# Renmusxd/PyIsingMonteCarlo

Measured on AMD Instinct MI355X. Metric: spin-flip attempts/s (whole node), 4096^2 2D Ising, higher is better.
Workload: dtype u32; 1 GPU; c2: 4096x4096 periodic Ising J=-1 beta=0.4407, 256 replicas/GPU, checkerboard Metropolis, bit-packed spins, Philox4x32-10; replicas_per_gpu=256, parallelism=replicas x1

## Files before the change

### pyisingmontecarlo_amd/csrc/lattice_kernels.hpp

```cpp
#pragma once
#include "philox.hpp"
#include <type_traits>

namespace isingmc {

struct LatGeom {
    uint32_t W, H;
    uint32_t wpr;
    uint32_t wpp;
    uint32_t nquads;
    int32_t cols_log2;
};

struct LatThr {
    uint64_t T3, T4;
};

#ifndef ISINGMC_N_PLANES
#define ISINGMC_N_PLANES 7
#endif
constexpr int N_PLANES = ISINGMC_N_PLANES;
constexpr int THR_BITS = N_PLANES + 32;

__device__ __forceinline__ uint32_t sel4(uint4 v, uint32_t i)
{
    return i == 0 ? v.x : i == 1 ? v.y : i == 2 ? v.z : v.w;
}

struct QuadNbr {
    uint32_t up[4], dn[4], ce[4], si[4];
};

template <bool UNI>
__device__ __forceinline__ void thread_to_quad(const LatGeom &g, uint32_t gid, uint32_t &Q, uint32_t &y,
                                               uint32_t &xw)
{
    if constexpr (UNI) {
        const uint32_t cl = uint32_t(g.cols_log2), col = gid & ((1u << cl) - 1);
        if (cl >= 6) {
            y = gid >> cl;
        } else {
            const uint32_t wave = gid >> 6, j = (gid & 63u) >> cl;
            y = ((wave >> 1) << (7 - cl)) + 2 * j + (wave & 1u);
        }
        Q = (y << cl) + col;
        xw = 4 * col;
    } else {
        Q = gid;
        y = (4 * Q) / g.wpr;
        xw = 4 * Q - y * g.wpr;
    }
}

struct PtrPlanes {
    uint32_t *own;
    const uint32_t *oth;
    __device__ __forceinline__ uint4 own4(uint32_t w) const { return *reinterpret_cast<const uint4 *>(own + w); }
    __device__ __forceinline__ uint4 oth4(uint32_t w) const { return *reinterpret_cast<const uint4 *>(oth + w); }
    __device__ __forceinline__ uint32_t own1(uint32_t w) const { return own[w]; }
    __device__ __forceinline__ uint32_t oth1(uint32_t w) const { return oth[w]; }
    __device__ __forceinline__ void store4(uint32_t w, uint4 v) const { *reinterpret_cast<uint4 *>(own + w) = v; }
    __device__ __forceinline__ void store1(uint32_t w, uint32_t v) const { own[w] = v; }
};

struct BufPlanes {
    __amdgpu_buffer_rsrc_t rsrc;
    uint32_t own_off, oth_off;
    typedef uint32_t u32x4 __attribute__((ext_vector_type(4)));
    __device__ __forceinline__ uint4 ld4(uint32_t byte_off) const
    {
        const u32x4 v = __builtin_amdgcn_raw_buffer_load_b128(rsrc, byte_off, 0, 0);
        return make_uint4(v.x, v.y, v.z, v.w);
    }
    __device__ __forceinline__ uint4 own4(uint32_t w) const { return ld4(own_off + 4 * w); }
    __device__ __forceinline__ uint4 oth4(uint32_t w) const { return ld4(oth_off + 4 * w); }
    __device__ __forceinline__ uint32_t own1(uint32_t w) const { return __builtin_amdgcn_raw_buffer_load_b32(rsrc, own_off + 4 * w, 0, 0); }
    __device__ __forceinline__ uint32_t oth1(uint32_t w) const { return __builtin_amdgcn_raw_buffer_load_b32(rsrc, oth_off + 4 * w, 0, 0); }
    __device__ __forceinline__ void store4(uint32_t w, uint4 v) const
    {
        __builtin_amdgcn_raw_buffer_store_b128(u32x4{v.x, v.y, v.z, v.w}, rsrc, own_off + 4 * w, 0, 0);
    }
    __device__ __forceinline__ void store1(uint32_t w, uint32_t v) const { __builtin_amdgcn_raw_buffer_store_b32(v, rsrc, own_off + 4 * w, 0, 0); }
};

__device__ __forceinline__ void side_words(QuadNbr &n, bool odd)
{
    const uint32_t sw = n.si[0];
    if (odd) {
        n.si[0] = (n.ce[0] >> 1) | (n.ce[1] << 31);
        n.si[1] = (n.ce[1] >> 1) | (n.ce[2] << 31);
        n.si[2] = (n.ce[2] >> 1) | (n.ce[3] << 31);
        n.si[3] = (n.ce[3] >> 1) | (sw << 31);
    } else {
        n.si[3] = (n.ce[3] << 1) | (n.ce[2] >> 31);
        n.si[2] = (n.ce[2] << 1) | (n.ce[1] >> 31);
        n.si[1] = (n.ce[1] << 1) | (n.ce[0] >> 31);
        n.si[0] = (n.ce[0] << 1) | (sw >> 31);
    }
}

template <bool VEC, bool UNI, typename Mem>
__device__ __forceinline__ void load_quad(const Mem &mem, const LatGeom &g,
                                          uint32_t colour, uint32_t Q, uint32_t y, uint32_t xw, uint32_t own[4],
                                          QuadNbr &n, uint32_t widx[4])
{
    if constexpr (VEC) {
        const uint32_t w0 = 4 * Q;
        const uint32_t yu = (y == 0 ? g.H : y) - 1, yd = (y + 1 == g.H) ? 0 : y + 1;
        bool odd = (y + colour) & 1u;
        if constexpr (UNI) odd = __builtin_amdgcn_readfirstlane(uint32_t(odd));
        const uint32_t sx = odd ? (xw + 4 == g.wpr ? 0 : xw + 4) : (xw == 0 ? g.wpr : xw) - 1;
        const auto row_base = [&](uint32_t row) { return UNI ? row << (uint32_t(g.cols_log2) + 2) : row * g.wpr; };
        const uint4 o4 = mem.own4(w0);
        const uint4 c4 = mem.oth4(w0);
        const uint4 u4 = mem.oth4(row_base(yu) + xw);
        const uint4 d4 = mem.oth4(row_base(yd) + xw);
        const uint32_t sw = mem.oth1(row_base(y) + sx);
        own[0] = o4.x; own[1] = o4.y; own[2] = o4.z; own[3] = o4.w;
        n.ce[0] = c4.x; n.ce[1] = c4.y; n.ce[2] = c4.z; n.ce[3] = c4.w;
        n.up[0] = u4.x; n.up[1] = u4.y; n.up[2] = u4.z; n.up[3] = u4.w;
        n.dn[0] = d4.x; n.dn[1] = d4.y; n.dn[2] = d4.z; n.dn[3] = d4.w;
        n.si[0] = sw;
        side_words(n, odd);
#pragma unroll
        for (int q = 0; q < 4; q++) widx[q] = w0 + q;
    } else {
#pragma unroll
        for (int q = 0; q < 4; q++) {
            const uint32_t w = 4 * Q + q;
            const uint32_t yy = w / g.wpr, xx = w - yy * g.wpr;
            const uint32_t yu = (yy == 0 ? g.H : yy) - 1, yd = (yy + 1 == g.H) ? 0 : yy + 1;
            const uint32_t row = yy * g.wpr;
            widx[q] = w;
            own[q] = mem.own1(w);
            n.ce[q] = mem.oth1(w);
            n.up[q] = mem.oth1(yu * g.wpr + xx);
            n.dn[q] = mem.oth1(yd * g.wpr + xx);
            if ((yy + colour) & 1) {
                const uint32_t nxt = mem.oth1(row + (xx + 1 == g.wpr ? 0 : xx + 1));
                n.si[q] = (n.ce[q] >> 1) | (nxt << 31);
            } else {
                const uint32_t prv = mem.oth1(row + (xx == 0 ? g.wpr : xx) - 1);
                n.si[q] = (n.ce[q] << 1) | (prv >> 31);
            }
        }
    }
}

template <bool PMJ>
__device__ __forceinline__ void bond_masks(const uint32_t own, const QuadNbr &n, int q,
                                           const uint32_t *__restrict__ jneg, uint32_t wpp,
                                           uint32_t widx, uint32_t jneg_uniform, uint32_t &a0,
                                           uint32_t &a1, uint32_t &a2, uint32_t &a3)
{
    if constexpr (PMJ) {
        a0 = own ^ n.up[q] ^ jneg[widx];
        a1 = own ^ n.dn[q] ^ jneg[wpp + widx];
        a2 = own ^ n.ce[q] ^ jneg[2 * wpp + widx];
        a3 = own ^ n.si[q] ^ jneg[3 * wpp + widx];
    } else {
        const uint32_t o = own ^ jneg_uniform;
        a0 = o ^ n.up[q];
        a1 = o ^ n.dn[q];
        a2 = o ^ n.ce[q];
        a3 = o ^ n.si[q];
    }
}

struct QuadState {
    uint32_t eq3[4], eq4[4], lt[4], und[4];
};

struct ThrBits {
    uint32_t hi3, hi4;
    uint32_t lo3, lo4;
    bool all3, all4;
    bool any_all;
};

__device__ __forceinline__ ThrBits thr_bits(const LatThr thr)
{
    ThrBits b;
    const uint32_t h3 = __builtin_amdgcn_readfirstlane(uint32_t(thr.T3 >> 32));
    const uint32_t h4 = __builtin_amdgcn_readfirstlane(uint32_t(thr.T4 >> 32));
    b.all3 = (h3 >> N_PLANES) != 0;
    b.all4 = (h4 >> N_PLANES) != 0;
    b.any_all = ((h3 | h4) >> N_PLANES) != 0;
    b.hi3 = h3 & ((1u << N_PLANES) - 1);
    b.hi4 = h4 & ((1u << N_PLANES) - 1);
    b.lo3 = uint32_t(thr.T3);
    b.lo4 = uint32_t(thr.T4);
    return b;
}

struct QuadSigns {
    uint32_t w[4][4];
};

template <bool PMJ>
__device__ __forceinline__ void load_signs(const uint32_t *__restrict__ jn, const LatGeom &g, const uint32_t Q, QuadSigns &js)
{
    if constexpr (PMJ) {
#pragma unroll
        for (int d = 0; d < 4; d++) {
            const uint4 v = *reinterpret_cast<const uint4 *>(jn + size_t(d) * g.wpp + 4 * size_t(Q));
            js.w[0][d] = v.x; js.w[1][d] = v.y; js.w[2][d] = v.z; js.w[3][d] = v.w;
        }
    }
}

template <bool PMJ>
__device__ __forceinline__ void quad_classes(const uint32_t own[4], const QuadNbr &n, const uint32_t widx[4], const LatGeom &g,
                                             const ThrBits &tb, const QuadSigns &js, const uint32_t jneg_uniform,
                                             QuadState &st)
{
#pragma unroll
    for (int q = 0; q < 4; q++) {
        uint32_t a0, a1, a2, a3;
        if constexpr (PMJ) {
            a0 = own[q] ^ n.up[q] ^ js.w[q][0];
            a1 = own[q] ^ n.dn[q] ^ js.w[q][1];
            a2 = own[q] ^ n.ce[q] ^ js.w[q][2];
            a3 = own[q] ^ n.si[q] ^ js.w[q][3];
        } else {
            bond_masks<false>(own[q], n, q, nullptr, g.wpp, widx[q], jneg_uniform, a0, a1, a2, a3);
        }
        const uint32_t s01 = a0 ^ a1, c01 = a0 & a1, s23 = a2 ^ a3, c23 = a2 & a3;
        st.eq4[q] = c01 & c23;
        st.eq3[q] = __builtin_amdgcn_bitop3_b32(c01, s23, c23 & s01, 0xEA);
        asm("" : "+v"(st.eq3[q]), "+v"(st.eq4[q]));
    }
    if (tb.any_all) {
#pragma unroll
        for (int q = 0; q < 4; q++) {
            if (tb.all3) st.eq3[q] = 0;
            if (tb.all4) st.eq4[q] = 0;
        }
    }
#pragma unroll
    for (int q = 0; q < 4; q++) {
        st.lt[q] = 0;
        st.und[q] = st.eq3[q] | st.eq4[q];
    }
}

__device__ __forceinline__ void plane_step(QuadState &st, const uint32_t rr[4], const int p, const ThrBits &tb)
{
    const auto step = [&](int q, uint32_t tbw) {
        st.lt[q] = __builtin_amdgcn_bitop3_b32(rr[q], tbw, st.lt[q], 0x8E);
        st.und[q] = __builtin_amdgcn_bitop3_b32(st.und[q], rr[q], tbw, 0x90);
    };
    const uint32_t sel = __builtin_amdgcn_readfirstlane(((tb.hi3 >> (N_PLANES - 1 - p)) & 1u) | (((tb.hi4 >> (N_PLANES - 1 - p)) & 1u) << 1));
    if (sel == 3) {
#pragma unroll
        for (int q = 0; q < 4; q++) step(q, st.eq3[q] | st.eq4[q]);
    } else if (sel == 1) {
#pragma unroll
        for (int q = 0; q < 4; q++) step(q, st.eq3[q]);
    } else if (sel == 2) {
#pragma unroll
        for (int q = 0; q < 4; q++) step(q, st.eq4[q]);
    } else {
#pragma unroll
        for (int q = 0; q < 4; q++) {
            st.lt[q] &= ~rr[q];
            st.und[q] &= ~rr[q];
        }
    }
}

template <int NQ>
__device__ __forceinline__ void quad_planes(QuadState (&st)[NQ], const uint32_t (&Q)[NQ], const uint32_t colour, const uint64_t t,
                                            const uint2 key, const PhiloxVKeys &vk, const ThrBits &tb)
{
    const uint32_t c0 = uint32_t(t);
#pragma unroll
    for (int p = N_PLANES - 1; p >= 0; p--) {
        uint32_t rr[NQ][4];
#pragma unroll
        for (int j = 0; j < NQ; j++) {
            const uint4 rnd = philox4x32_10(make_uint4(c0, Q[j], DOM_LAT_SWEEP, ctr2(t, colour, p)), key, vk);
            rr[j][0] = rnd.x; rr[j][1] = rnd.y; rr[j][2] = rnd.z; rr[j][3] = rnd.w;
        }
        auto step = [&](int j, int q, uint32_t tbw) {
            st[j].lt[q] = __builtin_amdgcn_bitop3_b32(rr[j][q], tbw, st[j].lt[q], 0x8E);
            st[j].und[q] = __builtin_amdgcn_bitop3_b32(st[j].und[q], rr[j][q], tbw, 0x90);
        };
        const uint32_t sel = __builtin_amdgcn_readfirstlane(((tb.hi3 >> (N_PLANES - 1 - p)) & 1u) | (((tb.hi4 >> (N_PLANES - 1 - p)) & 1u) << 1));
        if (sel == 3) {
#pragma unroll
            for (int j = 0; j < NQ; j++)
#pragma unroll
                for (int q = 0; q < 4; q++) step(j, q, st[j].eq3[q] | st[j].eq4[q]);
        } else if (sel == 1) {
#pragma unroll
            for (int j = 0; j < NQ; j++)
#pragma unroll
                for (int q = 0; q < 4; q++) step(j, q, st[j].eq3[q]);
        } else if (sel == 2) {
#pragma unroll
            for (int j = 0; j < NQ; j++)
#pragma unroll
                for (int q = 0; q < 4; q++) step(j, q, st[j].eq4[q]);
        } else {
#pragma unroll
            for (int j = 0; j < NQ; j++)
#pragma unroll
                for (int q = 0; q < 4; q++) {
                    st[j].lt[q] &= ~rr[j][q];
                    st[j].und[q] &= ~rr[j][q];
                }
        }
    }
}

struct QuadRandom {
    uint32_t rr[N_PLANES][4];
    uint4 tie;
};

__device__ __forceinline__ void quad_random(QuadRandom &R, const uint32_t Q, const uint32_t colour, const uint64_t t, const uint2 key,
                                            const PhiloxVKeys &vk)
{
    const uint32_t c0 = uint32_t(t);
#pragma unroll
    for (int p = 0; p < N_PLANES; p++) {
        const uint4 rnd = philox4x32_10(make_uint4(c0, Q, DOM_LAT_SWEEP, ctr2(t, colour, p)), key, vk);
        R.rr[p][0] = rnd.x; R.rr[p][1] = rnd.y; R.rr[p][2] = rnd.z; R.rr[p][3] = rnd.w;
    }
    R.tie = philox4x32_10(make_uint4(c0, Q, DOM_LAT_SWEEP, ctr2(t, colour, N_PLANES)), key, vk);
}

__device__ __forceinline__ void quad_ties(const QuadState &st, const uint32_t Q, const uint32_t colour, const uint64_t t,
                                          const uint2 key, const PhiloxVKeys &vk, const ThrBits &tb, uint32_t acc[4],
                                          const uint4 *first_call = nullptr)
{
    const uint32_t c0 = uint32_t(t), c1 = Q;
#pragma unroll
    for (int q = 0; q < 4; q++) acc[q] = __builtin_amdgcn_bitop3_b32(st.eq3[q], st.eq4[q], st.lt[q], 0xAB);
#ifdef ISINGMC_TIMING_ONLY_NO_TIES
    if (false) {
#else
    if (st.und[0] | st.und[1] | st.und[2] | st.und[3]) {
#endif
        const uint4 rnd = first_call ? *first_call : philox4x32_10(make_uint4(c0, c1, DOM_LAT_SWEEP, ctr2(t, colour, N_PLANES)), key, vk);
#ifdef ISINGMC_TIMING_ONLY_NO_TIE_LOOPS
        {
            const uint32_t rr4[4] = {rnd.x, rnd.y, rnd.z, rnd.w};
#pragma unroll
            for (int q = 0; q < 4; q++) acc[q] |= st.und[q] & (0u - uint32_t(rr4[q] < ((st.und[q] & st.eq4[q]) ? tb.lo4 : tb.lo3)));
            return;
        }
#endif
        const uint32_t n_ties = __popc(st.und[0]) + __popc(st.und[1]) + __popc(st.und[2]) + __popc(st.und[3]);
        if (n_ties <= 4) {
            uint32_t r0 = rnd.x, r1 = rnd.y, r2 = rnd.z, r3 = rnd.w;
            uint32_t lo3v, lo4v;
            asm volatile("v_mov_b32 %0, %1" : "=v"(lo3v) : "s"(tb.lo3));
            asm volatile("v_mov_b32 %0, %1" : "=v"(lo4v) : "s"(tb.lo4));
#pragma unroll
            for (int q = 0; q < 4; q++) {
                uint32_t m = st.und[q];
                while (m) {
                    const uint32_t bit = m & (0u - m);
                    m ^= bit;
                    const uint32_t lo = (bit & st.eq4[q]) ? lo4v : lo3v;
                    if (r0 < lo) acc[q] |= bit;
                    r0 = r1; r1 = r2; r2 = r3;
                }
            }
        } else {
            uint32_t nres = 0;
            uint4 w = rnd;
#pragma unroll
            for (int q = 0; q < 4; q++) {
                uint32_t m = st.und[q];
                while (m) {
                    const uint32_t b = __ffs(m) - 1;
                    m &= m - 1;
                    if (nres != 0 && (nres & 3u) == 0)
                        w = philox4x32_10(make_uint4(c0, c1, DOM_LAT_SWEEP, ctr2(t, colour, N_PLANES + (nres >> 2))), key, vk);
                    const uint32_t lo = ((st.eq4[q] >> b) & 1u) ? tb.lo4 : tb.lo3;
                    if (sel4(w, nres & 3u) < lo) acc[q] |= 1u << b;
                    nres++;
                }
            }
        }
    }
}

template <bool PMJ>
__device__ __forceinline__ void quad_flips(const uint32_t own[4], const QuadNbr &n, const uint32_t widx[4], const LatGeom &g,
                                           const uint32_t colour, const uint64_t t, const uint2 key, const PhiloxVKeys &vk,
                                           const LatThr thr, const QuadSigns &js, const uint32_t jneg_uniform,
                                           const uint32_t Q, uint32_t acc[4])
{
    const ThrBits tb = thr_bits(thr);
    QuadState st[1];
    const uint32_t Qs[1] = {Q};
    quad_classes<PMJ>(own, n, widx, g, tb, js, jneg_uniform, st[0]);
    quad_planes<1>(st, Qs, colour, t, key, vk, tb);
    quad_ties(st[0], Q, colour, t, key, vk, tb, acc);
}

template <bool PMJ>
__device__ __forceinline__ void quad_flips_pre(const uint32_t own[4], const QuadNbr &n, const uint32_t widx[4], const LatGeom &g,
                                               const uint32_t colour, const uint64_t t, const uint2 key, const PhiloxVKeys &vk,
                                               const LatThr thr, const QuadSigns &js, const uint32_t jneg_uniform, const uint32_t Q,
                                               const QuadRandom &R, uint32_t acc[4])
{
    const ThrBits tb = thr_bits(thr);
    QuadState st;
    quad_classes<PMJ>(own, n, widx, g, tb, js, jneg_uniform, st);
#pragma unroll
    for (int p = N_PLANES - 1; p >= 0; p--) plane_step(st, R.rr[p], p, tb);
    quad_ties(st, Q, colour, t, key, vk, tb, acc, &R.tie);
}

__device__ __forceinline__ void load_quad_uni(const BufPlanes &mem, const LatGeom &g, const uint32_t colour, const uint32_t gid,
                                              uint32_t &Q, uint32_t &vQ, uint32_t own[4], QuadNbr &n)
{
    typedef uint32_t u32x4 __attribute__((ext_vector_type(4)));
    const uint32_t cl = uint32_t(g.cols_log2), rb = 16u << cl;
    const uint32_t wave = __builtin_amdgcn_readfirstlane(gid >> 6), lane = gid & 63u;
    uint32_t y, col;
    bool lo_row, hi_row;
    uint32_t ypar;
    if (cl >= 6) {
        const uint32_t ys = wave >> (cl - 6);
        y = ys;
        col = gid & ((1u << cl) - 1);
        lo_row = ys == 0;
        hi_row = ys + 1 == g.H;
        ypar = ys & 1u;
    } else {
        const uint32_t rpw = 64u >> cl, ybase = ((wave >> 1) << (7 - cl)) + (wave & 1u);
        y = ybase + 2 * (lane >> cl);
        col = lane & ((1u << cl) - 1);
        lo_row = ybase == 0;
        hi_row = ybase + 2 * (rpw - 1) + 1 >= g.H;
        ypar = wave & 1u;
    }
    Q = (y << cl) + col;
    vQ = Q << 4;
    uint32_t vU, vD;
    if (lo_row | hi_row) {
        const uint32_t yu = (y == 0 ? g.H : y) - 1, yd = (y + 1 == g.H) ? 0 : y + 1;
        vU = ((yu << cl) + col) << 4;
        vD = ((yd << cl) + col) << 4;
    } else {
        vU = vQ - rb;
        vD = vQ + rb;
    }
    const bool odd = ((ypar + colour) & 1u) != 0;
    const uint32_t t16 = vQ & (rb - 1), rowb = vQ - t16;
    const uint32_t vS = rowb + (odd ? ((t16 + 16) & (rb - 1)) : ((t16 - 4) & (rb - 1)));
    const u32x4 o4 = __builtin_amdgcn_raw_buffer_load_b128(mem.rsrc, vQ, mem.own_off, 0);
    const u32x4 c4 = __builtin_amdgcn_raw_buffer_load_b128(mem.rsrc, vQ, mem.oth_off, 0);
    const u32x4 u4 = __builtin_amdgcn_raw_buffer_load_b128(mem.rsrc, vU, mem.oth_off, 0);
    const u32x4 d4 = __builtin_amdgcn_raw_buffer_load_b128(mem.rsrc, vD, mem.oth_off, 0);
    const uint32_t sw = __builtin_amdgcn_raw_buffer_load_b32(mem.rsrc, vS, mem.oth_off, 0);
    own[0] = o4.x; own[1] = o4.y; own[2] = o4.z; own[3] = o4.w;
    n.ce[0] = c4.x; n.ce[1] = c4.y; n.ce[2] = c4.z; n.ce[3] = c4.w;
    n.up[0] = u4.x; n.up[1] = u4.y; n.up[2] = u4.z; n.up[3] = u4.w;
    n.dn[0] = d4.x; n.dn[1] = d4.y; n.dn[2] = d4.z; n.dn[3] = d4.w;
    n.si[0] = sw;
    side_words(n, odd);
}

template <bool PMJ>
__device__ __forceinline__ void quad_measure(const uint32_t own_new[4], const QuadNbr &n, const QuadSigns &js,
                                             const uint32_t jneg_uniform, uint32_t &sat, uint32_t &up)
{
#pragma unroll
    for (int q = 0; q < 4; q++) {
        uint32_t a0, a1, a2, a3;
        if constexpr (PMJ) {
            a0 = own_new[q] ^ n.up[q] ^ js.w[q][0];
            a1 = own_new[q] ^ n.dn[q] ^ js.w[q][1];
            a2 = own_new[q] ^ n.ce[q] ^ js.w[q][2];
            a3 = own_new[q] ^ n.si[q] ^ js.w[q][3];
        } else {
            const uint32_t o = own_new[q] ^ jneg_uniform;
            a0 = o ^ n.up[q]; a1 = o ^ n.dn[q]; a2 = o ^ n.ce[q]; a3 = o ^ n.si[q];
        }
        sat += __popc(a0) + __popc(a1) + __popc(a2) + __popc(a3);
        (void)up;
    }
}

struct PendingQuad {
    uint32_t w[4];
    uint32_t widx[4];
};

template <bool VEC, typename Mem>
__device__ __forceinline__ void store_pending(const Mem &mem, const PendingQuad &p)
{
    if constexpr (VEC) {
        mem.store4(p.widx[0], make_uint4(p.w[0], p.w[1], p.w[2], p.w[3]));
    } else {
#pragma unroll
        for (int q = 0; q < 4; q++) mem.store1(p.widx[q], p.w[q]);
    }
}

template <bool VEC, bool PMJ, bool UNI, typename Mem, bool MEASURE = false>
__device__ __forceinline__ void update_quad(const Mem &mem, const LatGeom &g, const uint32_t colour, const uint64_t t, const uint2 key,
                                            const PhiloxVKeys &vk, const LatThr thr, const uint32_t *__restrict__ jn,
                                            const uint32_t jneg_uniform, const uint32_t gid, uint32_t *sat = nullptr,
                                            uint32_t *up = nullptr, PendingQuad *pending = nullptr)
{
    if constexpr (VEC && UNI && std::is_same<Mem, BufPlanes>::value) {
        typedef uint32_t u32x4 __attribute__((ext_vector_type(4)));
        uint32_t Q, vQ, own[4], acc[4];
        QuadNbr n;
        QuadSigns js;
        load_quad_uni(mem, g, colour, gid, Q, vQ, own, n);
        load_signs<PMJ>(jn, g, Q, js);
        const uint32_t widx[4] = {4 * Q, 4 * Q + 1, 4 * Q + 2, 4 * Q + 3};
        quad_flips<PMJ>(own, n, widx, g, colour, t, key, vk, thr, js, jneg_uniform, Q, acc);
        if constexpr (MEASURE) {
#pragma unroll
            for (int q = 0; q < 4; q++) { pending->w[q] = own[q] ^ acc[q]; pending->widx[q] = widx[q]; }
            quad_measure<PMJ>(pending->w, n, js, jneg_uniform, *sat, *up);
        } else {
            __builtin_amdgcn_raw_buffer_store_b128(u32x4{own[0] ^ acc[0], own[1] ^ acc[1], own[2] ^ acc[2], own[3] ^ acc[3]}, mem.rsrc,
                                                   vQ, mem.own_off, 0);
        }
        return;
    }
    uint32_t Q, qy, qxw;
    thread_to_quad<UNI>(g, gid, Q, qy, qxw);

    uint32_t own[4], widx[4], acc[4];
    QuadNbr n;
    QuadSigns js;
    load_signs<PMJ>(jn, g, Q, js);
    load_quad<VEC, UNI>(mem, g, colour, Q, qy, qxw, own, n, widx);
    quad_flips<PMJ>(own, n, widx, g, colour, t, key, vk, thr, js, jneg_uniform, Q, acc);

    if constexpr (MEASURE) {
#pragma unroll
        for (int q = 0; q < 4; q++) { pending->w[q] = own[q] ^ acc[q]; pending->widx[q] = widx[q]; }
        quad_measure<PMJ>(pending->w, n, js, jneg_uniform, *sat, *up);
    } else if constexpr (VEC) {
        mem.store4(widx[0], make_uint4(own[0] ^ acc[0], own[1] ^ acc[1], own[2] ^ acc[2], own[3] ^ acc[3]));
    } else {
#pragma unroll
        for (int q = 0; q < 4; q++) mem.store1(widx[q], own[q] ^ acc[q]);
    }
}

constexpr uint32_t MEASURE_SLOTS = 16;
#ifndef ISINGMC_MEASURE_WAVES
#define ISINGMC_MEASURE_WAVES 7
#endif

template <bool VEC, bool PMJ, bool UNI>
__global__ __launch_bounds__(256, ISINGMC_MEASURE_WAVES) void lat_sweep_measure_kernel(
    uint32_t *__restrict__ state, const LatGeom g, const uint64_t t, const uint2 *__restrict__ keys, const LatThr thr_uniform,
    const LatThr *__restrict__ thr_replica, const uint32_t *__restrict__ jneg, const uint32_t jneg_uniform,
    unsigned long long *__restrict__ out, const size_t out_stride)
{
    __shared__ uint32_t red[2][4];
    const uint32_t colour = 1;
    const uint32_t r = blockIdx.y;
    const uint32_t gid = blockIdx.x * 256 + threadIdx.x;
    uint32_t sat = 0, up = 0;
    BufPlanes mem;
    mem.rsrc = __builtin_amdgcn_make_buffer_rsrc(state + size_t(r) * 2 * g.wpp, 0, int(2 * g.wpp * sizeof(uint32_t)), 0x00020000);
    mem.own_off = colour * g.wpp * 4u;
    mem.oth_off = 0;
    PendingQuad pending;
    if (gid < g.nquads) {
        const uint2 key = keys[r];
        update_quad<VEC, PMJ, UNI, BufPlanes, true>(mem, g, colour, t, key, philox_vkeys(key), thr_replica ? thr_replica[r] : thr_uniform,
                                                    PMJ ? jneg + size_t(colour) * 4 * g.wpp : nullptr, jneg_uniform, gid, &sat, &up, &pending);
    }
#pragma unroll
    for (int off = 32; off > 0; off >>= 1) sat += __shfl_xor(sat, off);
    if ((threadIdx.x & 63) == 0) red[0][threadIdx.x >> 6] = sat;
    __syncthreads();
    if (threadIdx.x == 0) {
        unsigned long long *slot = out + size_t(r) * out_stride + 2 * (blockIdx.x % MEASURE_SLOTS);
        atomicAdd(slot, (unsigned long long)(red[0][0] + red[0][1] + red[0][2] + red[0][3]));
    }
    if (gid < g.nquads) store_pending<VEC>(mem, pending);
}

template <bool VEC, bool PMJ, bool UNI>
__global__ __launch_bounds__(256) void lat_sweep_kernel(
    uint32_t *__restrict__ state, const LatGeom g, const uint32_t colour, const uint64_t t,
    const uint2 *__restrict__ keys, const LatThr thr_uniform, const LatThr *__restrict__ thr_replica,
    const uint32_t *__restrict__ jneg, const uint32_t jneg_uniform)
{
    const uint32_t r = blockIdx.y;
    const uint32_t gid = blockIdx.x * 256 + threadIdx.x;
    if (gid >= g.nquads) return;
    BufPlanes mem;
    mem.rsrc = __builtin_amdgcn_make_buffer_rsrc(state + size_t(r) * 2 * g.wpp, 0, int(2 * g.wpp * sizeof(uint32_t)), 0x00020000);
    mem.own_off = colour * g.wpp * 4u;
    mem.oth_off = (1 - colour) * g.wpp * 4u;
    const uint2 key = keys[r];
    update_quad<VEC, PMJ, UNI>(mem, g, colour, t, key, philox_vkeys(key), thr_replica ? thr_replica[r] : thr_uniform,
                               PMJ ? jneg + size_t(colour) * 4 * g.wpp : nullptr, jneg_uniform, gid);
}

template <bool PMJ>
__global__ __launch_bounds__(256) void lat_sweep_loop_kernel(
    uint32_t *__restrict__ state, const LatGeom g, const uint32_t colour, const uint64_t t,
    const uint2 *__restrict__ keys, const LatThr thr_uniform, const LatThr *__restrict__ thr_replica,
    const uint32_t *__restrict__ jneg, const uint32_t jneg_uniform, const uint32_t iters)
{
    const uint32_t r = blockIdx.y;
    const uint32_t stride = gridDim.x * 256;
    uint32_t gid = blockIdx.x * 256 + threadIdx.x;
    BufPlanes mem;
    mem.rsrc = __builtin_amdgcn_make_buffer_rsrc(state + size_t(r) * 2 * g.wpp, 0, int(2 * g.wpp * sizeof(uint32_t)), 0x00020000);
    mem.own_off = colour * g.wpp * 4u;
    mem.oth_off = (1 - colour) * g.wpp * 4u;
    const uint2 key = keys[r];
    const PhiloxVKeys vk = philox_vkeys(key);
    const LatThr thr = thr_replica ? thr_replica[r] : thr_uniform;
    const uint32_t *jn = PMJ ? jneg + size_t(colour) * 4 * g.wpp : nullptr;
#pragma unroll 1
    for (uint32_t it = 0; it < iters; it++, gid += stride)
        update_quad<true, PMJ, true>(mem, g, colour, t, key, vk, thr, jn, jneg_uniform, gid);
}

__attribute__((unused)) static __global__ __launch_bounds__(256) void lat_init_kernel(uint32_t *__restrict__ state, const LatGeom g,
                                                       const uint2 *__restrict__ keys,
                                                       const uint32_t first_replica)
{
    const uint32_t r = first_replica + blockIdx.y;
    const uint32_t Q = blockIdx.x * 256 + threadIdx.x;
    if (Q >= 2 * g.nquads) return;
    const uint32_t c = Q >= g.nquads, q = Q - c * g.nquads;
    const uint4 rnd = philox4x32_10(make_uint4(0, q, ctr2(0, c, 0), DOM_LAT_INIT), keys[r]);
    *reinterpret_cast<uint4 *>(state + size_t(r) * 2 * g.wpp + size_t(c) * g.wpp + 4 * size_t(q)) = rnd;
}

constexpr uint32_t MEASURE_QUADS_PER_THREAD = 16;

template <bool VEC, bool PMJ>
__global__ __launch_bounds__(256) void lat_measure_kernel(
    const uint32_t *__restrict__ state, const LatGeom g, const uint32_t *__restrict__ jneg,
    const uint32_t jneg_uniform, unsigned long long *__restrict__ out, const size_t out_stride)
{
    __shared__ uint32_t red[2][4];
    const uint32_t r = blockIdx.y;
    uint32_t sat = 0, up = 0;
    const uint32_t *p0 = state + size_t(r) * 2 * g.wpp;
    for (uint32_t i = 0; i < MEASURE_QUADS_PER_THREAD; i++) {
        const uint32_t gid = (blockIdx.x * MEASURE_QUADS_PER_THREAD + i) * 256 + threadIdx.x;
        if (gid >= g.nquads) break;
        uint32_t Q, qy, qxw, own[4], widx[4];
        thread_to_quad<false>(g, gid, Q, qy, qxw);
        QuadNbr n;
        load_quad<VEC, false>(PtrPlanes{const_cast<uint32_t *>(p0), p0 + g.wpp}, g, 0, Q, qy, qxw, own, n, widx);
#pragma unroll
        for (int q = 0; q < 4; q++) {
            uint32_t a0, a1, a2, a3;
            bond_masks<PMJ>(own[q], n, q, jneg, g.wpp, widx[q], jneg_uniform, a0, a1, a2, a3);
            sat += __popc(a0) + __popc(a1) + __popc(a2) + __popc(a3);
            up += __popc(own[q]) + __popc(n.ce[q]);
        }
    }
#pragma unroll
    for (int off = 32; off > 0; off >>= 1) {
        sat += __shfl_xor(sat, off);
        up += __shfl_xor(up, off);
    }
    if ((threadIdx.x & 63) == 0) {
        red[0][threadIdx.x >> 6] = sat;
        red[1][threadIdx.x >> 6] = up;
    }
    __syncthreads();
    if (threadIdx.x == 0) {
        atomicAdd(out + size_t(r) * out_stride, (unsigned long long)(red[0][0] + red[0][1] + red[0][2] + red[0][3]));
        atomicAdd(out + size_t(r) * out_stride + 1, (unsigned long long)(red[1][0] + red[1][1] + red[1][2] + red[1][3]));
    }
}

constexpr uint32_t LDS_RESIDENT_MAX_BYTES = 64 * 1024;

template <bool VEC, bool PMJ>
__global__ __launch_bounds__(1024) void lat_resident_kernel(
    uint32_t *__restrict__ state, const LatGeom g, const uint64_t t0, const uint32_t timesteps,
    const uint2 *__restrict__ keys, const LatThr *__restrict__ thr_steps, const uint32_t thr_stride,
    const LatThr *__restrict__ thr_replica, const uint32_t *__restrict__ jneg, const uint32_t jneg_uniform,
    unsigned long long *__restrict__ steps_out, const uint32_t n_replicas)
{
    extern __shared__ __attribute__((aligned(16))) uint32_t planes[];
    __shared__ uint32_t red[2][16];
    const uint32_t r = blockIdx.x, tid = threadIdx.x, nthreads = blockDim.x;
    uint32_t *mine = state + size_t(r) * 2 * g.wpp;
    for (uint32_t i = tid; i < g.wpp / 2; i += nthreads)
        reinterpret_cast<uint4 *>(planes)[i] = reinterpret_cast<const uint4 *>(mine)[i];
    const uint2 key = keys[r];
    const PhiloxVKeys vk = philox_vkeys(key);
    __syncthreads();
    for (uint32_t k = 0; k < timesteps; k++) {
        const LatThr thr = thr_replica ? thr_replica[r] : thr_steps[size_t(k) * thr_stride];
        for (uint32_t colour = 0; colour < 2; colour++) {
            for (uint32_t gid = tid; gid < g.nquads; gid += nthreads)
                update_quad<VEC, PMJ, false>(PtrPlanes{planes + colour * g.wpp, planes + (1 - colour) * g.wpp}, g, colour, t0 + k,
                                             key, vk, thr, PMJ ? jneg + size_t(colour) * 4 * g.wpp : nullptr, jneg_uniform,
                                             gid);
            __syncthreads();
        }
        if (steps_out) {
            uint32_t sat = 0, up = 0;
            for (uint32_t gid = tid; gid < g.nquads; gid += nthreads) {
                uint32_t Q, qy, qxw, own[4], widx[4];
                thread_to_quad<false>(g, gid, Q, qy, qxw);
                QuadNbr n;
                load_quad<VEC, false>(PtrPlanes{planes, planes + g.wpp}, g, 0, Q, qy, qxw, own, n, widx);
#pragma unroll
                for (int q = 0; q < 4; q++) {
                    uint32_t a0, a1, a2, a3;
                    bond_masks<PMJ>(own[q], n, q, jneg, g.wpp, widx[q], jneg_uniform, a0, a1, a2, a3);
                    sat += __popc(a0) + __popc(a1) + __popc(a2) + __popc(a3);
                    up += __popc(own[q]) + __popc(n.ce[q]);
                }
            }
#pragma unroll
            for (int off = 32; off > 0; off >>= 1) {
                sat += __shfl_xor(sat, off);
                up += __shfl_xor(up, off);
            }
            if ((tid & 63) == 0) { red[0][tid >> 6] = sat; red[1][tid >> 6] = up; }
            __syncthreads();
            if (tid == 0) {
                unsigned long long s = 0, u = 0;
                for (uint32_t w = 0; w < (nthreads + 63) / 64; w++) { s += red[0][w]; u += red[1][w]; }
                steps_out[(size_t(k) * n_replicas + r) * 2] = s;
                steps_out[(size_t(k) * n_replicas + r) * 2 + 1] = u;
            }
            __syncthreads();
        }
    }
    for (uint32_t i = tid; i < g.wpp / 2; i += nthreads)
        reinterpret_cast<uint4 *>(mine)[i] = reinterpret_cast<const uint4 *>(planes)[i];
}

__attribute__((unused)) static __global__ void lat_energy_from_counts_kernel(unsigned long long *__restrict__ meas, const uint32_t n,
                                              const double jabs, const long long n_bonds, double *__restrict__ out)
{
    const uint32_t r = blockIdx.x * blockDim.x + threadIdx.x;
    if (r < n) {
        out[r] = jabs * double(n_bonds - 2 * (long long)meas[2 * size_t(r)]);
        meas[2 * size_t(r)] = 0;
        meas[2 * size_t(r) + 1] = 0;
    }
}

}
```

Baseline: 10000 billion spin-flip attempts/s.

## Stream Metropolis acceptance planes MSB-first with scalar-selected threshold paths

```diff
diff --git a/pyisingmontecarlo_amd/csrc/lattice_kernels.hpp b/pyisingmontecarlo_amd/csrc/lattice_kernels.hpp
--- a/pyisingmontecarlo_amd/csrc/lattice_kernels.hpp
+++ b/pyisingmontecarlo_amd/csrc/lattice_kernels.hpp
@@ -331,13 +331,15 @@
     R.tie = philox4x32_10(make_uint4(c0, Q, DOM_LAT_SWEEP, ctr2(t, colour, N_PLANES)), key, vk);
 }
 
+template <bool WORD = false>
 __device__ __forceinline__ void quad_ties(const QuadState &st, const uint32_t Q, const uint32_t colour, const uint64_t t,
                                           const uint2 key, const PhiloxVKeys &vk, const ThrBits &tb, uint32_t acc[4],
                                           const uint4 *first_call = nullptr)
 {
     const uint32_t c0 = uint32_t(t), c1 = Q;
 #pragma unroll
-    for (int q = 0; q < 4; q++) acc[q] = __builtin_amdgcn_bitop3_b32(st.eq3[q], st.eq4[q], st.lt[q], 0xAB);
+    for (int q = 0; q < 4; q++)
+        if constexpr (!WORD) acc[q] = __builtin_amdgcn_bitop3_b32(st.eq3[q], st.eq4[q], st.lt[q], 0xAB);
 #ifdef ISINGMC_TIMING_ONLY_NO_TIES
     if (false) {
 #else
@@ -348,7 +350,7 @@
         {
             const uint32_t rr4[4] = {rnd.x, rnd.y, rnd.z, rnd.w};
 #pragma unroll
-            for (int q = 0; q < 4; q++) acc[q] |= st.und[q] & (0u - uint32_t(rr4[q] < ((st.und[q] & st.eq4[q]) ? tb.lo4 : tb.lo3)));
+            for (int q = 0; q < 4; q++) acc[q] ^= st.und[q] & (0u - uint32_t(rr4[q] < ((st.und[q] & st.eq4[q]) ? tb.lo4 : tb.lo3)));
             return;
         }
 #endif
@@ -365,7 +367,8 @@
                     const uint32_t bit = m & (0u - m);
                     m ^= bit;
                     const uint32_t lo = (bit & st.eq4[q]) ? lo4v : lo3v;
-                    if (r0 < lo) acc[q] |= bit;
+                    if constexpr (WORD) { if (r0 < lo) acc[q] ^= bit; }
+                    else { if (r0 < lo) acc[q] |= bit; }
                     r0 = r1; r1 = r2; r2 = r3;
                 }
             }
@@ -381,7 +384,8 @@
                     if (nres != 0 && (nres & 3u) == 0)
                         w = philox4x32_10(make_uint4(c0, c1, DOM_LAT_SWEEP, ctr2(t, colour, N_PLANES + (nres >> 2))), key, vk);
                     const uint32_t lo = ((st.eq4[q] >> b) & 1u) ? tb.lo4 : tb.lo3;
-                    if (sel4(w, nres & 3u) < lo) acc[q] |= 1u << b;
+                    if constexpr (WORD) { if (sel4(w, nres & 3u) < lo) acc[q] ^= 1u << b; }
+                    else { if (sel4(w, nres & 3u) < lo) acc[q] |= 1u << b; }
                     nres++;
                 }
             }
@@ -468,6 +472,183 @@
     side_words(n, odd);
 }
 
+
+__device__ __forceinline__ void wave_rows(const LatGeom &g, const uint32_t wave, bool &edge, uint32_t &ypar)
+{
+    const uint32_t cl = uint32_t(g.cols_log2);
+    if (cl >= 6) {
+        const uint32_t ys = wave >> (cl - 6);
+        edge = ys == 0 || ys + 1 == g.H;
+        ypar = ys & 1u;
+    } else {
+        const uint32_t rpw = 64u >> cl, ybase = ((wave >> 1) << (7 - cl)) + (wave & 1u);
+        edge = ybase == 0 || ybase + 2 * (rpw - 1) + 1 >= g.H;
+        ypar = wave & 1u;
+    }
+}
+
+struct QuadAddr {
+    uint32_t Q, vQ, vU, vD, vS;
+};
+
+__device__ __forceinline__ uint32_t quad_of_thread(const LatGeom &g, const uint32_t gid, const uint32_t wave)
+{
+    const uint32_t cl = uint32_t(g.cols_log2);
+    if (cl >= 6) return gid;
+    const uint32_t lane = gid & 63u, ybase = ((wave >> 1) << (7 - cl)) + (wave & 1u);
+    return ((ybase + 2 * (lane >> cl)) << cl) + (lane & ((1u << cl) - 1));
+}
+
+__device__ __forceinline__ void quad_addr(const LatGeom &g, const bool edge, const bool odd, QuadAddr &a)
+{
+    const uint32_t cl = uint32_t(g.cols_log2), rb = 16u << cl;
+    a.vQ = a.Q << 4;
+    if (edge) {
+        const uint32_t y = a.Q >> cl, col = a.Q & ((1u << cl) - 1);
+        const uint32_t yu = (y == 0 ? g.H : y) - 1, yd = (y + 1 == g.H) ? 0 : y + 1;
+        a.vU = ((yu << cl) + col) << 4;
+        a.vD = ((yd << cl) + col) << 4;
+    } else {
+        a.vU = a.vQ - rb;
+        a.vD = a.vQ + rb;
+    }
+    const uint32_t t16 = a.vQ & (rb - 1), rowb = a.vQ - t16;
+    a.vS = rowb + (odd ? ((t16 + 16) & (rb - 1)) : ((t16 - 4) & (rb - 1)));
+}
+
+__device__ __forceinline__ void load_quad_at(const BufPlanes &mem, const QuadAddr &a, const uint32_t soff, const bool odd,
+                                             uint32_t own[4], QuadNbr &n)
+{
+    typedef uint32_t u32x4 __attribute__((ext_vector_type(4)));
+    const uint32_t so = mem.own_off + soff, sn = mem.oth_off + soff;
+    const u32x4 o4 = __builtin_amdgcn_raw_buffer_load_b128(mem.rsrc, a.vQ, so, 0);
+    const u32x4 c4 = __builtin_amdgcn_raw_buffer_load_b128(mem.rsrc, a.vQ, sn, 0);
+    const u32x4 u4 = __builtin_amdgcn_raw_buffer_load_b128(mem.rsrc, a.vU, sn, 0);
+    const u32x4 d4 = __builtin_amdgcn_raw_buffer_load_b128(mem.rsrc, a.vD, sn, 0);
+    const uint32_t sw = __builtin_amdgcn_raw_buffer_load_b32(mem.rsrc, a.vS, sn, 0);
+    own[0] = o4.x; own[1] = o4.y; own[2] = o4.z; own[3] = o4.w;
+    n.ce[0] = c4.x; n.ce[1] = c4.y; n.ce[2] = c4.z; n.ce[3] = c4.w;
+    n.up[0] = u4.x; n.up[1] = u4.y; n.up[2] = u4.z; n.up[3] = u4.w;
+    n.dn[0] = d4.x; n.dn[1] = d4.y; n.dn[2] = d4.z; n.dn[3] = d4.w;
+    n.si[0] = sw;
+    side_words(n, odd);
+}
+
+__device__ __forceinline__ ThrBits thr_bits_scalar(const LatThr thr)
+{
+    ThrBits b = thr_bits(thr);
+    b.lo3 = __builtin_amdgcn_readfirstlane(b.lo3);
+    b.lo4 = __builtin_amdgcn_readfirstlane(b.lo4);
+    return b;
+}
+
+template <bool PMJ>
+__device__ __forceinline__ void stream_classes(const uint32_t own[4], const QuadNbr &n, const ThrBits &tb, const QuadSigns &js,
+                                               const uint32_t jneg_uniform, QuadState &st, uint32_t x[4])
+{
+    const auto classes = [&](const int q, const uint32_t up, const uint32_t dn, const uint32_t ce, const uint32_t si, const bool neg) {
+        const uint32_t c01 = neg ? __builtin_amdgcn_bitop3_b32(own[q], up, dn, 0x81) : __builtin_amdgcn_bitop3_b32(own[q], up, dn, 0x18);
+        const uint32_t c23 = neg ? __builtin_amdgcn_bitop3_b32(own[q], ce, si, 0x81) : __builtin_amdgcn_bitop3_b32(own[q], ce, si, 0x18);
+        const uint32_t u = __builtin_amdgcn_bitop3_b32(c01, ce, si, 0x60);
+        const uint32_t v = __builtin_amdgcn_bitop3_b32(c23, up, dn, 0x60);
+        st.eq4[q] = c01 & c23;
+        st.eq3[q] = u | v;
+    };
+    if constexpr (PMJ) {
+#pragma unroll
+        for (int q = 0; q < 4; q++)
+            classes(q, n.up[q] ^ js.w[q][0], n.dn[q] ^ js.w[q][1], n.ce[q] ^ js.w[q][2], n.si[q] ^ js.w[q][3], false);
+    } else if (jneg_uniform) {
+#pragma unroll
+        for (int q = 0; q < 4; q++) classes(q, n.up[q], n.dn[q], n.ce[q], n.si[q], true);
+    } else {
+#pragma unroll
+        for (int q = 0; q < 4; q++) classes(q, n.up[q], n.dn[q], n.ce[q], n.si[q], false);
+    }
+#pragma unroll
+    for (int q = 0; q < 4; q++) asm("" : "+v"(st.eq3[q]), "+v"(st.eq4[q]));
+    if (tb.any_all) {
+#pragma unroll
+        for (int q = 0; q < 4; q++) {
+            if (tb.all3) st.eq3[q] = 0;
+            if (tb.all4) st.eq4[q] = 0;
+        }
+    }
+#pragma unroll
+    for (int q = 0; q < 4; q++) x[q] = __builtin_amdgcn_bitop3_b32(own[q], st.eq3[q], st.eq4[q], 0xE1);
+}
+
+template <uint32_t TT_LT, uint32_t TT_UND>
+__device__ __forceinline__ void first_plane(QuadState &st, const uint32_t rr[4])
+{
+#pragma unroll
+    for (int q = 0; q < 4; q++) {
+        if constexpr (TT_LT == 0) st.lt[q] = 0;
+        else st.lt[q] = __builtin_amdgcn_bitop3_b32(rr[q], st.eq3[q], st.eq4[q], TT_LT);
+        st.und[q] = __builtin_amdgcn_bitop3_b32(rr[q], st.eq3[q], st.eq4[q], TT_UND);
+    }
+}
+
+__device__ __forceinline__ void stream_planes(QuadState &st, const uint32_t Q, const uint32_t colour, const uint64_t t, const uint2 key,
+                                              const PhiloxVKeys &vk, const ThrBits &tb)
+{
+    const uint32_t c0 = uint32_t(t);
+#pragma unroll
+    for (int p = N_PLANES - 1; p >= 0; p--) {
+        const uint4 rnd = philox4x32_10(make_uint4(c0, Q, DOM_LAT_SWEEP, ctr2(t, colour, p)), key, vk);
+        const uint32_t rr[4] = {rnd.x, rnd.y, rnd.z, rnd.w};
+        const uint32_t sel = __builtin_amdgcn_readfirstlane(((tb.hi3 >> (N_PLANES - 1 - p)) & 1u) | (((tb.hi4 >> (N_PLANES - 1 - p)) & 1u) << 1));
+        if (p == N_PLANES - 1) {
+            if (sel == 3) first_plane<0x0E, 0xE0>(st, rr);
+            else if (sel == 1) first_plane<0x0C, 0xC2>(st, rr);
+            else if (sel == 2) first_plane<0x0A, 0xA4>(st, rr);
+            else first_plane<0x00, 0x0E>(st, rr);
+            continue;
+        }
+        const auto step = [&](const int q, const uint32_t tbw) {
+            st.lt[q] = __builtin_amdgcn_bitop3_b32(rr[q], tbw, st.lt[q], 0x8E);
+            st.und[q] = __builtin_amdgcn_bitop3_b32(st.und[q], rr[q], tbw, 0x90);
+        };
+        if (sel == 3) {
+#pragma unroll
+            for (int q = 0; q < 4; q++) step(q, st.eq3[q] | st.eq4[q]);
+        } else if (sel == 1) {
+#pragma unroll
+            for (int q = 0; q < 4; q++) step(q, st.eq3[q]);
+        } else if (sel == 2) {
+#pragma unroll
+            for (int q = 0; q < 4; q++) step(q, st.eq4[q]);
+        } else {
+#pragma unroll
+            for (int q = 0; q < 4; q++) {
+                st.lt[q] &= ~rr[q];
+                st.und[q] &= ~rr[q];
+            }
+        }
+    }
+}
+
+template <bool PMJ>
+__device__ __forceinline__ void stream_update_quad(const BufPlanes &mem, const LatGeom &g, const uint32_t colour, const uint64_t t,
+                                                   const uint2 key, const PhiloxVKeys &vk, const ThrBits &tb,
+                                                   const uint32_t *__restrict__ jn, const uint32_t jneg_uniform, const QuadAddr &a,
+                                                   const uint32_t soff, const bool odd)
+{
+    typedef uint32_t u32x4 __attribute__((ext_vector_type(4)));
+    uint32_t own[4], w[4];
+    QuadNbr n;
+    QuadSigns js;
+    load_quad_at(mem, a, soff, odd, own, n);
+    load_signs<PMJ>(jn, g, a.Q, js);
+    QuadState st;
+    stream_classes<PMJ>(own, n, tb, js, jneg_uniform, st, w);
+    stream_planes(st, a.Q, colour, t, key, vk, tb);
+#pragma unroll
+    for (int q = 0; q < 4; q++) w[q] ^= st.lt[q];
+    quad_ties<true>(st, a.Q, colour, t, key, vk, tb, w);
+    __builtin_amdgcn_raw_buffer_store_b128(u32x4{w[0], w[1], w[2], w[3]}, mem.rsrc, a.vQ, mem.own_off + soff, 0);
+}
+
 template <bool PMJ>
 __device__ __forceinline__ void quad_measure(const uint32_t own_new[4], const QuadNbr &n, const QuadSigns &js,
                                              const uint32_t jneg_uniform, uint32_t &sat, uint32_t &up)
@@ -511,8 +692,19 @@
                                             const uint32_t jneg_uniform, const uint32_t gid, uint32_t *sat = nullptr,
                                             uint32_t *up = nullptr, PendingQuad *pending = nullptr)
 {
+    if constexpr (VEC && UNI && std::is_same<Mem, BufPlanes>::value && !MEASURE) {
+        const uint32_t wave = __builtin_amdgcn_readfirstlane(gid >> 6);
+        bool edge;
+        uint32_t ypar;
+        wave_rows(g, wave, edge, ypar);
+        const bool odd = ((ypar + colour) & 1u) != 0;
+        QuadAddr a;
+        a.Q = quad_of_thread(g, gid, wave);
+        quad_addr(g, edge, odd, a);
+        stream_update_quad<PMJ>(mem, g, colour, t, key, vk, thr_bits_scalar(thr), jn, jneg_uniform, a, 0, odd);
+        return;
+    }
     if constexpr (VEC && UNI && std::is_same<Mem, BufPlanes>::value) {
-        typedef uint32_t u32x4 __attribute__((ext_vector_type(4)));
         uint32_t Q, vQ, own[4], acc[4];
         QuadNbr n;
         QuadSigns js;
@@ -520,14 +712,9 @@
         load_signs<PMJ>(jn, g, Q, js);
         const uint32_t widx[4] = {4 * Q, 4 * Q + 1, 4 * Q + 2, 4 * Q + 3};
         quad_flips<PMJ>(own, n, widx, g, colour, t, key, vk, thr, js, jneg_uniform, Q, acc);
-        if constexpr (MEASURE) {
-#pragma unroll
-            for (int q = 0; q < 4; q++) { pending->w[q] = own[q] ^ acc[q]; pending->widx[q] = widx[q]; }
-            quad_measure<PMJ>(pending->w, n, js, jneg_uniform, *sat, *up);
-        } else {
-            __builtin_amdgcn_raw_buffer_store_b128(u32x4{own[0] ^ acc[0], own[1] ^ acc[1], own[2] ^ acc[2], own[3] ^ acc[3]}, mem.rsrc,
-                                                   vQ, mem.own_off, 0);
-        }
+#pragma unroll
+        for (int q = 0; q < 4; q++) { pending->w[q] = own[q] ^ acc[q]; pending->widx[q] = widx[q]; }
+        quad_measure<PMJ>(pending->w, n, js, jneg_uniform, *sat, *up);
         return;
     }
     uint32_t Q, qy, qxw;
@@ -607,26 +794,73 @@
                                PMJ ? jneg + size_t(colour) * 4 * g.wpp : nullptr, jneg_uniform, gid);
 }
 
-template <bool PMJ>
-__global__ __launch_bounds__(256) void lat_sweep_loop_kernel(
+template <bool PMJ, bool PROBE>
+__device__ __forceinline__ void sweep_loop_body(
     uint32_t *__restrict__ state, const LatGeom g, const uint32_t colour, const uint64_t t,
     const uint2 *__restrict__ keys, const LatThr thr_uniform, const LatThr *__restrict__ thr_replica,
-    const uint32_t *__restrict__ jneg, const uint32_t jneg_uniform, const uint32_t iters)
+    const uint32_t *__restrict__ jneg, const uint32_t jneg_uniform, const uint32_t iters, const uint32_t stride)
 {
     const uint32_t r = blockIdx.y;
-    const uint32_t stride = gridDim.x * 256;
-    uint32_t gid = blockIdx.x * 256 + threadIdx.x;
+    const uint32_t gid = blockIdx.x * 256 + threadIdx.x;
     BufPlanes mem;
     mem.rsrc = __builtin_amdgcn_make_buffer_rsrc(state + size_t(r) * 2 * g.wpp, 0, int(2 * g.wpp * sizeof(uint32_t)), 0x00020000);
     mem.own_off = colour * g.wpp * 4u;
     mem.oth_off = (1 - colour) * g.wpp * 4u;
     const uint2 key = keys[r];
     const PhiloxVKeys vk = philox_vkeys(key);
-    const LatThr thr = thr_replica ? thr_replica[r] : thr_uniform;
+    ThrBits tb = thr_bits_scalar(thr_replica ? thr_replica[r] : thr_uniform);
+    if constexpr (PROBE) {
+        static_assert(!PROBE || N_PLANES == 7, "the probe's threshold bits are those of 7 planes");
+        tb.hi3 = 21;
+        tb.hi4 = 3;
+        tb.all3 = tb.all4 = tb.any_all = false;
+    }
     const uint32_t *jn = PMJ ? jneg + size_t(colour) * 4 * g.wpp : nullptr;
+    const uint32_t cl = uint32_t(g.cols_log2);
+    const bool parity_flips = cl >= 6 && ((stride >> cl) & 1u) != 0;
+    uint32_t wave = __builtin_amdgcn_readfirstlane(gid >> 6);
+    bool edge;
+    uint32_t ypar;
+    wave_rows(g, wave, edge, ypar);
+    if constexpr (PROBE) __builtin_assume(!edge);
+    bool odd = ((ypar + colour) & 1u) != 0;
+    QuadAddr a;
+    a.Q = quad_of_thread(g, gid, wave);
+    quad_addr(g, edge, odd, a);
+    uint32_t soff = 0;
 #pragma unroll 1
-    for (uint32_t it = 0; it < iters; it++, gid += stride)
-        update_quad<true, PMJ, true>(mem, g, colour, t, key, vk, thr, jn, jneg_uniform, gid);
+    for (uint32_t it = 0; it < iters; it++) {
+        stream_update_quad<PMJ>(mem, g, colour, t, key, vk, tb, jn, jneg_uniform, a, soff, odd);
+        a.Q += stride;
+        wave += stride >> 6;
+        bool edge_next;
+        wave_rows(g, wave, edge_next, ypar);
+        if constexpr (PROBE) __builtin_assume(!edge_next);
+        const bool redo = edge | edge_next | parity_flips;
+        edge = edge_next;
+        odd = ((ypar + colour) & 1u) != 0;
+        if (redo) {
+            quad_addr(g, true, odd, a);
+            soff = 0;
+        } else {
+            soff += stride << 4;
+        }
+    }
+}
+
+template <bool PMJ>
+__global__ __launch_bounds__(256) void lat_sweep_loop_kernel(
+    uint32_t *__restrict__ state, const LatGeom g, const uint32_t colour, const uint64_t t,
+    const uint2 *__restrict__ keys, const LatThr thr_uniform, const LatThr *__restrict__ thr_replica,
+    const uint32_t *__restrict__ jneg, const uint32_t jneg_uniform, const uint32_t iters)
+{
+#ifdef ISINGMC_ISA_BUDGET_PROBE
+    (void)g; (void)thr_replica; (void)jneg_uniform; (void)iters;
+    sweep_loop_body<PMJ, true>(state, LatGeom{4096, 4096, 64, 4096 * 64, 4096 * 16, 4}, colour, t, keys, thr_uniform, nullptr, jneg, 0u, 2u,
+                               4096u * 16u / 2u);
+#else
+    sweep_loop_body<PMJ, false>(state, g, colour, t, keys, thr_uniform, thr_replica, jneg, jneg_uniform, iters, gridDim.x * 256);
+#endif
 }
 
 __attribute__((unused)) static __global__ __launch_bounds__(256) void lat_init_kernel(uint32_t *__restrict__ state, const LatGeom g,
```

Result: slower. 9891 billion spin-flip attempts/s (-1.1%).
